# Meng-333/SRADSGAN

Measured on AMD Instinct MI355X. Metric: training images/sec (216x216, x4), higher is better.
Workload: dtype f32 (split-bf16 products: 3 bf16 MFMA terms per fp32 multiply, fp32 accumulate)

## Files before the change

### include/sradsgan_hip.h

```cpp
#ifndef SRADSGAN_HIP_H
#define SRADSGAN_HIP_H
#include <stddef.h>
#include <stdint.h>

#ifdef __cplusplus
extern "C" {
#endif

#define SRHIP_OK 0
#define SRHIP_ERR_ARG (-1)
#define SRHIP_ERR_LAUNCH (-2)
#define SRHIP_ERR_WORKSPACE (-3)

#define SRHIP_EPI_BIAS 1
#define SRHIP_EPI_LRELU 2
#define SRHIP_EPI_RESIDUAL 4
#define SRHIP_EPI_ROWSCALE 8
#define SRHIP_EPI_ACTMASK 32
#define SRHIP_EPI_CHANSCALE 16
#define SRHIP_EPI_GRADDATA 64

const char* srhip_last_error(void);
int srhip_abi_version(void);
int srhip_stream_fork(void* from_stream, void* to_stream);
// ... 178 lines not shown
size_t srhip_attn_tail_bwd_workspace(int n, int h, int w);
int srhip_attn_tail_bwd_spatial(const float* dz, const float* u, const float* s, const float* m, const float* pooled,
                                const int* argc, const float* w7, float* du, float* ds, float* dw7, int accumulate_dw7,
                                void* workspace, size_t workspace_bytes, int n, int h, int w, int c, void* stream);
size_t srhip_attn_tail_mlp_workspace(int n, int hidden);
int srhip_attn_tail_bwd_mlp(const float* ds, const float* avg, const float* mx, const float* s, const float* fc1,
                            const float* fc2, float* davg, float* dmax, float* dfc1, float* dfc2, int accumulate_dfc,
                            void* workspace, size_t workspace_bytes, int n, int c, int hidden, void* stream);
size_t srhip_attn_tail_bwd_fused_workspace(int n, int h, int w, int hidden);
int srhip_attn_tail_bwd(const float* dz, const float* u, const float* s, const float* m, const float* pooled, const int* argc,
                        const float* avg, const float* mx, const int* argmax_hw, const float* w7, const float* fc1,
                        const float* fc2, float* du, float* dw7, int accumulate_dw7, float* dfc1, float* dfc2,
                        int accumulate_dfc, void* workspace, size_t workspace_bytes, int n, int h, int w, int c, int hidden,
                        void* stream);
int srhip_attn_tail_bwd_pp(const float* dz, const float* u, const float* s, const float* m, const float* pooled, const int* argc,
                        const float* avg, const float* mx, const int* argmax_hw, const float* w7, const float* fc1,
                        const float* fc2, float* du, void* du_pp, float* dw7, int accumulate_dw7, float* dfc1, float* dfc2,
                        int accumulate_dfc, void* workspace, size_t workspace_bytes, int n, int h, int w, int c, int hidden,
                        void* stream);
int srhip_attn_tail_bwd_channel(float* du, const float* davg, const float* dmax, const int* argmax_hw, int n, int h,
                                int w, int c, void* stream);

size_t srhip_cgam_workspace(int n, int hw);
int srhip_cgam_fwd(const float* x, const float* gamma, float* y, float* att, void* workspace, size_t workspace_bytes,
                   int n, int hw, int c, void* stream);
int srhip_cgam_bwd(const float* dy, const float* x, const float* att, const float* gamma, float* dx, float* dgamma,
                   int accumulate_dgamma, void* workspace, size_t workspace_bytes, int n, int hw, int c, void* stream);
int srhip_sgam_flash_fwd(const float* q, const float* k, const float* v, const float* x, const float* gamma, float* y,
                         float* o, float* lse, int n, int hw, int dk, int c, void* stream);
size_t srhip_sgam_flash_bwd_workspace(int n, int hw);
int srhip_sgam_flash_bwd(const float* dy, const float* q, const float* k, const float* v, const float* o, const float* lse,
                         const float* gamma, float* dq, float* dk_out, float* dv, float* dgamma, int accumulate_dgamma,
                         void* workspace, size_t workspace_bytes, int n, int hw, int dk, int c, void* stream);

int srhip_cbam_pool_hw(const float* x, float* t, int* arg, int fixed_arg, int n, int hw, int c, void* stream);
int srhip_cbam_unpool_hw(const float* t, const int* arg, float* out, int n, int hw, int c, void* stream);
int srhip_cbam_pool_c(const float* x, float* t, int* argc, int fixed_arg, int n, int hw, int c, void* stream);
int srhip_cbam_unpool_c(const float* t, const int* argc, float* out, int n, int hw, int c, void* stream);
int srhip_cbam_scale(const float* x, const float* s, float* out, int n, int hw, int c, int mode, void* stream);
int srhip_cbam_dot(const float* a, const float* b, float* out, int n, int hw, int c, int mode, void* stream);
int srhip_sigmoid_fwd(const float* x, float* y, long count, int c, int pair, void* stream);
int srhip_sigmoid_bwd(const float* g, const float* y, float* dx, long count, int c, int pair, void* stream);
int srhip_sigmoid_bwd_bwd(const float* gg, const float* g, const float* y, float* dg, float* dy, long count, int c, int pair,
                          void* stream);

size_t srhip_reduce_workspace(void);
int srhip_l1_mean_fwd(const float* a, const float* b, float* out, void* workspace, size_t workspace_bytes, long count,
                      void* stream);
int srhip_l1_mean_bwd(const float* a, const float* b, const float* gout, float* da, float* db, long count, void* stream);
int srhip_mse_mean_fwd(const float* a, const float* b, float* out, void* workspace, size_t workspace_bytes, long count,
                       void* stream);
int srhip_mse_mean_bwd(const float* a, const float* b, const float* gout, float* da, float* db, long count, void* stream);
int srhip_smooth_l1_mean_fwd(const float* a, const float* b, float target, float* out, void* workspace, size_t workspace_bytes,
                             long count, void* stream);
int srhip_smooth_l1_mean_bwd(const float* a, const float* b, float target, const float* gout, float* da, float* db, long count,
                             void* stream);
int srhip_mean_fwd(const float* x, float* out, void* workspace, size_t workspace_bytes, long count, void* stream);
int srhip_mean_bwd(const float* gout, float* dx, long count, void* stream);
int srhip_gp_norm_penalty_fwd(const float* grads, float* out, void* workspace, size_t workspace_bytes, long npix, int c,
                              void* stream);
int srhip_gp_norm_penalty_bwd(const float* grads, const float* gout, float* dgrads, long npix, int c, void* stream);
#define SRHIP_GP_NORM_L2 0
#define SRHIP_GP_NORM_L1 1
#define SRHIP_GP_NORM_LINF 2
#define SRHIP_GP_PENALTY_LS 0
#define SRHIP_GP_PENALTY_HINGE 1
// ... 87 lines not shown
```

### sradsgan_amd/_hip.py

```python
import ctypes
import os

_HERE = os.path.dirname(os.path.abspath(__file__))
LIB_PATH = os.path.join(_HERE, 'lib', 'libsradsgan_hip.so')

_vp, _i, _f, _l, _sz = ctypes.c_void_p, ctypes.c_int, ctypes.c_float, ctypes.c_long, ctypes.c_size_t

SIGNATURES = {
    'srhip_last_error': (ctypes.c_char_p, []),
    'srhip_abi_version': (_i, []),
    'srhip_stream_fork': (_i, [_vp, _vp]),
    'srhip_debug_set': (_i, [_i, _i]),
    'srhip_probe_config': (_i, [_i] * 7),
    'srhip_probe_read': (_i, [_vp, _vp, _i]),
    'srhip_set_conv_math': (_i, [_i]),
    'srhip_get_conv_math': (_i, []),
    'srhip_resample_ksize': (_i, [_i, _i, _i]),
    'srhip_resample_coeffs': (_i, [_i, _i, _i, _vp, _vp]),
    'srhip_resample_pass_u8': (_i, [_vp, _vp, _vp, _vp, _i, _i, _i, _i, _i, _i, _i, _vp]),
    'srhip_u8_to_float': (_i, [_vp, _vp, _l, _vp]),
    'srhip_scene_tiles_u8': (_i, [_vp, _i, _i, _vp, _i, _i, _i, _vp, _vp]),
    'srhip_scene_blend_u8': (_i, [_vp, _i, _l, _l, _l] + [_vp] * 6 + [_i] * 8 + [_vp] * 3),
    'srhip_packed_elems': (_sz, [_i] * 5),
    'srhip_pack_entry_bytes': (_i, []),
# ... 23 lines not shown
    'srhip_conv2d_wgrad_pp_workspace': (_sz, [_i] * 8),
    'srhip_conv2d_wgrad_pp': (_i, [_i, _vp, _vp, _i, _i, _vp, _vp, _i, _vp, _sz] + [_i] * 6 + [_vp]),
    'srhip_conv2d_wgrad_act_ok': (_i, [_i] * 9),
    'srhip_conv2d_wgrad_act': (_i, [_vp] * 3 + [_f] + [_vp] * 3 + [_sz] + [_i] * 11 + [_vp]),
    'srhip_conv2d_wgrad': (_i, [_vp] * 6 + [_i, _vp, _sz] + [_i] * 11 + [_vp]),
    'srhip_colsum_workspace': (_sz, [_l, _i]),
    'srhip_colsum': (_i, [_vp, _vp, _vp, _sz, _l, _i, _i, _vp]),
    'srhip_lrelu_bwd': (_i, [_vp, _vp, _vp, _l, _f, _vp]),
    'srhip_lrelu_mask_bytes': (_sz, [_l]),
    'srhip_lrelu_bwd_bits': (_i, [_vp, _vp, _vp, _vp, _l, _f, _vp]),
    'srhip_maxpool2x2_fwd': (_i, [_vp, _vp, _i, _i, _i, _i, _vp]),
    'srhip_maxpool2x2_bwd': (_i, [_vp, _vp, _vp, _i, _i, _i, _i, _i, _vp]),
    'srhip_maxpool2x2_fwd_idx': (_i, [_vp, _vp, _vp, _i, _i, _i, _i, _vp]),
    'srhip_maxpool2x2_bwd_idx': (_i, [_vp, _vp, _vp, _i, _i, _i, _i, _i, _vp]),
    'srhip_pixel_shuffle_fwd': (_i, [_vp, _vp, _i, _i, _i, _i, _i, _f, _i, _vp]),
    'srhip_pixel_shuffle_bwd': (_i, [_vp, _vp, _vp, _i, _i, _i, _i, _i, _f, _i, _vp]),
    'srhip_attn_tail_workspace': (_sz, [_i]),
    'srhip_attn_tail_fwd': (_i, [_vp] * 12 + [_sz] + [_i] * 5 + [_vp]),
    'srhip_attn_tail_eval': (_i, [_vp] * 9 + [_sz] + [_i] * 5 + [_vp]),
    'srhip_attn_tail_bwd_workspace': (_sz, [_i] * 3),
    'srhip_attn_tail_bwd_spatial': (_i, [_vp] * 10 + [_i, _vp, _sz] + [_i] * 4 + [_vp]),
    'srhip_attn_tail_mlp_workspace': (_sz, [_i, _i]),
    'srhip_attn_tail_bwd_mlp': (_i, [_vp] * 10 + [_i, _vp, _sz] + [_i] * 3 + [_vp]),
    'srhip_attn_tail_bwd_fused_workspace': (_sz, [_i] * 4),
    'srhip_attn_tail_bwd': (_i, [_vp] * 14 + [_i] + [_vp] * 2 + [_i, _vp, _sz] + [_i] * 5 + [_vp]),
    'srhip_attn_tail_bwd_pp': (_i, [_vp] * 15 + [_i] + [_vp] * 2 + [_i, _vp, _sz] + [_i] * 5 + [_vp]),
    'srhip_attn_tail_bwd_channel': (_i, [_vp] * 4 + [_i] * 4 + [_vp]),
    'srhip_cgam_workspace': (_sz, [_i, _i]),
    'srhip_cgam_fwd': (_i, [_vp] * 5 + [_sz] + [_i] * 3 + [_vp]),
    'srhip_cgam_bwd': (_i, [_vp] * 6 + [_i, _vp, _sz] + [_i] * 3 + [_vp]),
    'srhip_sgam_flash_fwd': (_i, [_vp] * 8 + [_i] * 4 + [_vp]),
    'srhip_sgam_flash_bwd_workspace': (_sz, [_i, _i]),
    'srhip_sgam_flash_bwd': (_i, [_vp] * 11 + [_i, _vp, _sz] + [_i] * 4 + [_vp]),
    'srhip_cbam_pool_hw': (_i, [_vp, _vp, _vp, _i, _i, _i, _i, _vp]),
    'srhip_cbam_unpool_hw': (_i, [_vp, _vp, _vp, _i, _i, _i, _vp]),
    'srhip_cbam_pool_c': (_i, [_vp, _vp, _vp, _i, _i, _i, _i, _vp]),
    'srhip_cbam_unpool_c': (_i, [_vp, _vp, _vp, _i, _i, _i, _vp]),
    'srhip_cbam_scale': (_i, [_vp, _vp, _vp, _i, _i, _i, _i, _vp]),
    'srhip_cbam_dot': (_i, [_vp, _vp, _vp, _i, _i, _i, _i, _vp]),
    'srhip_sigmoid_fwd': (_i, [_vp, _vp, _l, _i, _i, _vp]),
    'srhip_sigmoid_bwd': (_i, [_vp, _vp, _vp, _l, _i, _i, _vp]),
    'srhip_sigmoid_bwd_bwd': (_i, [_vp] * 5 + [_l, _i, _i, _vp]),
    'srhip_reduce_workspace': (_sz, []),
    'srhip_l1_mean_fwd': (_i, [_vp] * 4 + [_sz, _l, _vp]),
    'srhip_l1_mean_bwd': (_i, [_vp] * 5 + [_l, _vp]),
    'srhip_mse_mean_fwd': (_i, [_vp] * 4 + [_sz, _l, _vp]),
    'srhip_mse_mean_bwd': (_i, [_vp] * 5 + [_l, _vp]),
    'srhip_smooth_l1_mean_fwd': (_i, [_vp, _vp, _f, _vp, _vp, _sz, _l, _vp]),
    'srhip_smooth_l1_mean_bwd': (_i, [_vp, _vp, _f] + [_vp] * 3 + [_l, _vp]),
    'srhip_mean_fwd': (_i, [_vp] * 3 + [_sz, _l, _vp]),
    'srhip_mean_bwd': (_i, [_vp] * 2 + [_l, _vp]),
    'srhip_gp_norm_penalty_fwd': (_i, [_vp] * 3 + [_sz, _l, _i, _vp]),
    'srhip_gp_norm_penalty_bwd': (_i, [_vp] * 3 + [_l, _i, _vp]),
    'srhip_gp_penalty_fwd': (_i, [_vp] * 3 + [_sz, _l, _i, _i, _i, _vp]),
    'srhip_gp_penalty_bwd': (_i, [_vp] * 3 + [_l, _i, _i, _i, _vp]),
    'srhip_bn_eval_fwd': (_i, [_vp] * 6 + [_l, _i, _f, _f, _i, _vp]),
    'srhip_dp_id_bytes': (_i, []),
    'srhip_dp_unique_id': (_i, [_vp]),
    'srhip_dp_init': (_i, [_vp, _i, _i]),
    'srhip_dp_world': (_i, []),
    'srhip_dp_rank': (_i, []),
    'srhip_dp_allreduce_bucket': (_i, [_vp, _sz, _vp]),
    'srhip_dp_broadcast': (_i, [_vp, _sz, _i, _vp]),
    'srhip_dp_finalize': (_i, []),
    'srhip_bn_workspace': (_sz, [_l, _i]),
    'srhip_bn_train_fwd': (_i, [_vp] * 9 + [_sz, _l, _i, _f, _f, _f, _i, _vp]),
# ... 109 lines not shown
```

### sradsgan_amd/csrc/global_attn.hip

```cpp
#include <math.h>

#include "common.h"

namespace srhip {

__device__ inline f32x16 ga_mfma(float a, float b, f32x16 c) { return __builtin_amdgcn_mfma_f32_32x32x2f32(a, b, c, 0, 0, 0); }
__device__ __forceinline__ int ga_row(int r, int h) { return (r & 3) + 8 * (r >> 2) + 4 * h; }

constexpr int GA_C = 64;
constexpr int GA_PIX = 128;
constexpr int GA_MS = 65;
constexpr int GA_VS = 68;
constexpr int GA_DK = 8;

__global__ __launch_bounds__(256) void ga_gram_partial_kernel(const float* __restrict__ a, const float* __restrict__ bm,
                                                              float* __restrict__ part, int hw, int nsplit) {
  const int split = blockIdx.x, img = blockIdx.y;
  const int lane = threadIdx.x & 63, wave = threadIdx.x >> 6;
  const int qi = wave >> 1, qj = wave & 1, h = lane >> 5, l31 = lane & 31;
  const int p0 = split * GA_PIX, p1 = min(p0 + GA_PIX, hw);
  const float* ab = a + (size_t)img * hw * GA_C + qi * 32 + l31;
  const float* bb = bm + (size_t)img * hw * GA_C + qj * 32 + l31;
  f32x16 acc;
#pragma unroll
  for (int r = 0; r < 16; ++r) acc[r] = 0.f;
  for (int p = p0; p < p1; p += 16) {
    float av[8], bv[8];
#pragma unroll
    for (int s = 0; s < 8; ++s) {
      const int pp = p + 2 * s + h;
      const bool ok = pp < p1;
      av[s] = ok ? ab[(size_t)pp * GA_C] : 0.f;
      bv[s] = ok ? bb[(size_t)pp * GA_C] : 0.f;
    }
#pragma unroll
// ... 793 lines not shown
    }
#pragma unroll
    for (int s = 0; s < 2; ++s) {
      ga_bf16x8 ph, pl;
      ga_split_regs(p, s, ph, pl);
#pragma unroll
      for (int u = 0; u < 2; ++u) {
        const int off = (32 * u + l31) * GA_TS + 16 * s + 8 * h;
        dvt[u] = ga_mma3(GA_FRAG(dth[b] + off), GA_FRAG(dtl[b] + off), ph, pl, dvt[u]);
      }
    }
#pragma unroll
    for (int r = 0; r < 16; ++r) p[r] = p[r] * (dp[r] - dd[r]);
#pragma unroll
    for (int s = 0; s < 2; ++s) {
      ga_bf16x8 sh, sl2;
      ga_split_regs(p, s, sh, sl2);
      const int off = (l31 & 7) * GA_TS + 16 * s + 8 * h;
      dkt = ga_mma3(GA_FRAG(qth[b] + off), GA_FRAG(qtl[b] + off), sh, sl2, dkt);
    }
    if (t + 1 < nt) store(b ^ 1);
    __syncthreads();
  }
  if (!kvalid) return;
  *reinterpret_cast<float4*>(dk + (base + kj) * GA_DK + 4 * h) = make_float4(dkt[0], dkt[1], dkt[2], dkt[3]);
#pragma unroll
  for (int u = 0; u < 2; ++u)
#pragma unroll
    for (int gq = 0; gq < 4; ++gq)
      *reinterpret_cast<float4*>(dv + (base + kj) * GA_C + 32 * u + 8 * gq + 4 * h) =
          make_float4(dvt[u][4 * gq], dvt[u][4 * gq + 1], dvt[u][4 * gq + 2], dvt[u][4 * gq + 3]);
}

int g_sgam_cfg = 0;
static inline bool ga_split_math() { return g_conv_math >= 1 && g_sgam_cfg != 1; }

static inline int ga_nsplit(int hw) { return cdiv(hw, GA_PIX); }
static inline int ga_prep_blocks(long npix) {
  long b = (npix + 15) / 16;
  return (int)(b < 1 ? 1 : (b > 1024 ? 1024 : b));
}

}

using namespace srhip;

extern "C" {

size_t srhip_cgam_workspace(int n, int hw) {
  if (n <= 0 || hw <= 0) return 0;
  return ((size_t)n * ga_nsplit(hw) * GA_C * GA_C + (size_t)n * GA_C * GA_C + (size_t)n + 64) * sizeof(float);
}

int srhip_cgam_fwd(const float* x, const float* gamma, float* y, float* att, void* workspace, size_t workspace_bytes,
                   int n, int hw, int c, void* stream) {
  SRHIP_REQUIRE(c == GA_C, "cgam_fwd: C must be 64 (sradsgan.py:194), got %d", c);
  SRHIP_REQUIRE(n > 0 && hw > 0, "cgam_fwd: empty input");
  SRHIP_REQUIRE((((uintptr_t)x | (uintptr_t)y | (uintptr_t)att) & 15) == 0, "cgam_fwd: pointers must be 16-byte aligned");
  if (!workspace || workspace_bytes < srhip_cgam_workspace(n, hw)) {
    set_error("cgam_fwd: workspace %zu bytes < required %zu", workspace_bytes, srhip_cgam_workspace(n, hw));
    return SRHIP_ERR_WORKSPACE;
  }
  hipStream_t st = as_stream(stream);
  const int ns = ga_nsplit(hw);
  float* part = static_cast<float*>(workspace);
  hipLaunchKernelGGL(ga_gram_partial_kernel, dim3(ns, n), dim3(256), 0, st, x, x, part, hw, ns);
// ... 41 lines not shown
  const long npix = (long)n * hw;
  return ((size_t)npix + (size_t)ga_prep_blocks(npix) + 64) * sizeof(float);
}

int srhip_sgam_flash_bwd(const float* dy, const float* q, const float* k, const float* v, const float* o, const float* lse,
                         const float* gamma, float* dq, float* dk_, float* dv, float* dgamma, int accumulate_dgamma,
                         void* workspace, size_t workspace_bytes, int n, int hw, int dk, int c, void* stream) {
  SRHIP_REQUIRE(c == GA_C && dk == GA_DK, "sgam_flash_bwd: C must be 64 and q/k channels 8, got %d / %d", c, dk);
  SRHIP_REQUIRE(n > 0 && hw > 0, "sgam_flash_bwd: empty input");
  SRHIP_REQUIRE((((uintptr_t)q | (uintptr_t)k | (uintptr_t)v | (uintptr_t)dy | (uintptr_t)o | (uintptr_t)dq | (uintptr_t)dk_ | (uintptr_t)dv) & 15) == 0,
                "sgam_flash_bwd: pointers must be 16-byte aligned");
  if (!workspace || workspace_bytes < srhip_sgam_flash_bwd_workspace(n, hw)) {
    set_error("sgam_flash_bwd: workspace %zu bytes < required %zu", workspace_bytes, srhip_sgam_flash_bwd_workspace(n, hw));
    return SRHIP_ERR_WORKSPACE;
  }
  hipStream_t st = as_stream(stream);
  const long npix = (long)n * hw;
  const int pb = ga_prep_blocks(npix);
  float* rowdot = static_cast<float*>(workspace);
  float* dgpart = rowdot + npix;
  hipLaunchKernelGGL(ga_sgam_bwd_prep_kernel, dim3(pb), dim3(256), 0, st, dy, o, rowdot, dgpart, npix);
  if (dgamma) hipLaunchKernelGGL(ga_sum_small_kernel, dim3(1), dim3(64), 0, st, dgpart, pb, dgamma, accumulate_dgamma);
  const dim3 grid(cdiv(hw, GA_PIX), n);
  if (ga_split_math()) {
    hipLaunchKernelGGL(ga_sgam_bwd_dq_x3_kernel, grid, dim3(256), 0, st, q, k, v, dy, lse, rowdot, gamma, dq, hw);
    hipLaunchKernelGGL(ga_sgam_bwd_dkv_x3_kernel, grid, dim3(256), 0, st, q, k, v, dy, lse, rowdot, gamma, dk_, dv, hw);
  } else {
    hipLaunchKernelGGL(ga_sgam_bwd_dq_kernel, grid, dim3(256), 0, st, q, k, v, dy, lse, rowdot, gamma, dq, hw);
    hipLaunchKernelGGL(ga_sgam_bwd_dkv_kernel, grid, dim3(256), 0, st, q, k, v, dy, lse, rowdot, gamma, dk_, dv, hw);
  }
  return check_launch("sgam_flash_bwd");
}

}
```

### sradsgan_amd/ops.py

```python
import contextlib
import ctypes
import os
import threading
import weakref
from typing import NamedTuple

import torch
from torch.autograd import Function

from . import _hip

EPI_BIAS, EPI_LRELU, EPI_RESIDUAL, EPI_ROWSCALE, EPI_CHANSCALE, EPI_GRADDATA = 1, 2, 4, 8, 16, 64
CL = torch.channels_last

class _State:
    skip_param_grads = False
    wgrads = None
    skip_ids = frozenset()
    stop_ids = frozenset()
    capturing = False
    last_out_pp = None
    carry = None
    carry_expect = None
    carry_token = 0
# ... 1577 lines not shown

    @staticmethod
    def backward(ctx, dy):
        x, att, gamma = ctx.saved_tensors
        dy = nhwc(dy)
        n, c, h, w = x.shape
        lib = _hip.lib()
        dx = torch.empty_like(x, memory_format=CL)
        skip = _skip_param_grads(gamma) or not ctx.needs_input_grad[1]
        dgam, acc = (None, 0) if skip else _gamma_slot(gamma)
        ws = _ws(lib.srhip_cgam_workspace(n, h * w), x)
        gam = gamma.detach().reshape(1).contiguous()
        _hip.check(lib.srhip_cgam_bwd(_p(dy), _p(x), _p(att), _p(gam), _p(dx), _p(dgam), acc, _p(ws), ws.numel() * 4,
                                      n, h * w, c, _stream()), 'cgam_bwd')
        return dx, (None if (skip or acc) else dgam.view(gamma.shape))


def cgam(x, gamma):
    return _Cgam.apply(x, gamma)


class _SgamCore(Function):

    @staticmethod
    def forward(ctx, x, q, k, v, gamma):
        _require_gpu(x, 'sgam')
        x, q, k, v = nhwc(x), nhwc(q), nhwc(k), nhwc(v)
        n, c, h, w = x.shape
        lib = _hip.lib()
        y = torch.empty_like(x, memory_format=CL)
        o = torch.empty_like(x, memory_format=CL)
        lse = torch.empty(n, h * w, device=x.device, dtype=torch.float32)
        gam = gamma.detach().reshape(1).contiguous()
        _hip.check(lib.srhip_sgam_flash_fwd(_p(q), _p(k), _p(v), _p(x), _p(gam), _p(y), _p(o), _p(lse), n, h * w,
                                            q.shape[1], c, _stream()), 'sgam_flash_fwd')
        ctx.save_for_backward(q, k, v, o, lse, gamma)
        return y

    @staticmethod
    def backward(ctx, dy):
        q, k, v, o, lse, gamma = ctx.saved_tensors
        dy = nhwc(dy)
        n, c, h, w = v.shape
        lib = _hip.lib()
        dq, dk = torch.empty_like(q, memory_format=CL), torch.empty_like(k, memory_format=CL)
        dv = torch.empty_like(v, memory_format=CL)
        skip = _skip_param_grads(gamma) or not ctx.needs_input_grad[4]
        dgam, acc = (None, 0) if skip else _gamma_slot(gamma)
        ws = _ws(lib.srhip_sgam_flash_bwd_workspace(n, h * w), v)
        gam = gamma.detach().reshape(1).contiguous()
        _hip.check(lib.srhip_sgam_flash_bwd(_p(dy), _p(q), _p(k), _p(v), _p(o), _p(lse), _p(gam), _p(dq), _p(dk), _p(dv),
                                            _p(dgam), acc, _p(ws), ws.numel() * 4, n, h * w, q.shape[1], c, _stream()),
                   'sgam_flash_bwd')
        return _passed_through(dy), dq, dk, dv, (None if (skip or acc) else dgam.view(gamma.shape))


def sgam(x, q, k, v, gamma):
    return _SgamCore.apply(x, q, k, v, gamma)


def _bn_reference_bwd(dy, x, y, gamma, eps, slope):
    n = x.numel() // x.shape[1]
    dz = dy if slope is None else dy * torch.where(y > 0, 1.0, float(slope))
    mean = x.mean((0, 2, 3), keepdim=True)
    var = x.var((0, 2, 3), unbiased=False, keepdim=True)
    invstd = torch.rsqrt(var + eps)
    xhat = (x - mean) * invstd
    dbeta = dz.sum((0, 2, 3))
    dgamma = (dz * xhat).sum((0, 2, 3))
    dx = (gamma.view(1, -1, 1, 1) * invstd) * (dz - dbeta.view(1, -1, 1, 1) / n - xhat * dgamma.view(1, -1, 1, 1) / n)
    return dx, dgamma, dbeta


_BN_BWD_X = os.environ.get('SRHIP_BN_BWD_X', '1') == '1'
_BN_FOLD = os.environ.get('SRHIP_BN_FOLD', '1') == '1'


@contextlib.contextmanager
def bn_fold_second_order():
    if not _BN_FOLD:
        yield
        return
    prev, _state.bn_fold = getattr(_state, 'bn_fold', None), {}
    ok = False
    try:
        yield
# ... 1322 lines not shown
```

Before: 673.6.

## Stage pre-split K/V tile images via LDS DMA in spatial attention kernels

Adds a pre-pass that packs each 32-pixel key/value tile into a contiguous global "image" holding both the fp32 data and the bf16 hi/lo split operands. The spatial-attention forward and backward kernels then stream these images into LDS with double-buffered buffer-load DMA, instead of each block re-splitting and transposing K/V itself. The intent is to drop the redundant per-block split/transpose work and to overlap global loads with MFMA compute. The cost is extra workspace, extra image-build launches and more global traffic for the packed tiles.

```diff
diff --git a/include/sradsgan_hip.h b/include/sradsgan_hip.h
--- a/include/sradsgan_hip.h
+++ b/include/sradsgan_hip.h
@@ -234,6 +234,14 @@
 int srhip_sgam_flash_bwd(const float* dy, const float* q, const float* k, const float* v, const float* o, const float* lse,
                          const float* gamma, float* dq, float* dk_out, float* dv, float* dgamma, int accumulate_dgamma,
                          void* workspace, size_t workspace_bytes, int n, int hw, int dk, int c, void* stream);
+size_t srhip_sgam_staged_fwd_workspace(int n, int hw);
+int srhip_sgam_staged_fwd(const float* q, const float* k, const float* v, const float* x, const float* gamma, float* y,
+                          float* o, float* lse, void* workspace, size_t workspace_bytes, int n, int hw, int dk, int c,
+                          void* stream);
+size_t srhip_sgam_staged_bwd_workspace(int n, int hw);
+int srhip_sgam_staged_bwd(const float* dy, const float* q, const float* k, const float* v, const float* o, const float* lse,
+                          const float* gamma, float* dq, float* dk_out, float* dv, float* dgamma, int accumulate_dgamma,
+                          void* workspace, size_t workspace_bytes, int n, int hw, int dk, int c, void* stream);
 
 int srhip_cbam_pool_hw(const float* x, float* t, int* arg, int fixed_arg, int n, int hw, int c, void* stream);
 int srhip_cbam_unpool_hw(const float* t, const int* arg, float* out, int n, int hw, int c, void* stream);
diff --git a/sradsgan_amd/_hip.py b/sradsgan_amd/_hip.py
--- a/sradsgan_amd/_hip.py
+++ b/sradsgan_amd/_hip.py
@@ -79,6 +79,10 @@
     'srhip_sgam_flash_fwd': (_i, [_vp] * 8 + [_i] * 4 + [_vp]),
     'srhip_sgam_flash_bwd_workspace': (_sz, [_i, _i]),
     'srhip_sgam_flash_bwd': (_i, [_vp] * 11 + [_i, _vp, _sz] + [_i] * 4 + [_vp]),
+    'srhip_sgam_staged_fwd_workspace': (_sz, [_i, _i]),
+    'srhip_sgam_staged_fwd': (_i, [_vp] * 9 + [_sz] + [_i] * 4 + [_vp]),
+    'srhip_sgam_staged_bwd_workspace': (_sz, [_i, _i]),
+    'srhip_sgam_staged_bwd': (_i, [_vp] * 11 + [_i, _vp, _sz] + [_i] * 4 + [_vp]),
     'srhip_cbam_pool_hw': (_i, [_vp, _vp, _vp, _i, _i, _i, _i, _vp]),
     'srhip_cbam_unpool_hw': (_i, [_vp, _vp, _vp, _i, _i, _i, _vp]),
     'srhip_cbam_pool_c': (_i, [_vp, _vp, _vp, _i, _i, _i, _i, _vp]),
diff --git a/sradsgan_amd/csrc/global_attn.hip b/sradsgan_amd/csrc/global_attn.hip
--- a/sradsgan_amd/csrc/global_attn.hip
+++ b/sradsgan_amd/csrc/global_attn.hip
@@ -1,6 +1,7 @@
 #include <math.h>
 
 #include "common.h"
+#include "conv_dev.h"
 
 namespace srhip {
 
@@ -860,6 +861,338 @@
           make_float4(dvt[u][4 * gq], dvt[u][4 * gq + 1], dvt[u][4 * gq + 2], dvt[u][4 * gq + 3]);
 }
 
+constexpr int GI_KT = 0;
+constexpr int GF_VTH = 1024, GF_VTL = GF_VTH + GA_C * GA_TS * 2, GF_TILE = GF_VTL + GA_C * GA_TS * 2;
+constexpr int GQ_KTH = 1024, GQ_KTL = GQ_KTH + GA_DK * GA_TS * 2, GQ_VRH = GQ_KTL + GA_DK * GA_TS * 2,
+              GQ_VRL = GQ_VRH + 32 * GA_RS * 2, GQ_END = GQ_VRL + 32 * GA_RS * 2, GQ_TILE = 12288;
+constexpr int GK_QTH = 1024, GK_QTL = GK_QTH + GA_DK * GA_TS * 2, GK_LT = GK_QTL + GA_DK * GA_TS * 2, GK_DT = GK_LT + 128,
+              GK_DRH = GK_DT + 128, GK_DRL = GK_DRH + 32 * GA_RS * 2, GK_DTH = GK_DRL + 32 * GA_RS * 2,
+              GK_DTL = GK_DTH + GA_C * GA_TS * 2, GK_END = GK_DTL + GA_C * GA_TS * 2, GK_TILE = 22528;
+static_assert(GF_TILE % 1024 == 0 && GQ_TILE % 1024 == 0 && GK_TILE % 1024 == 0, "a wave's DMA moves 1 KB");
+static_assert(GQ_END <= GQ_TILE && GK_END <= GK_TILE, "image layout");
+
+template <int KIND>
+__global__ __launch_bounds__(256) void ga_sgam_image_kernel(const float* __restrict__ wide, const float* __restrict__ narrow,
+                                                            const float* __restrict__ lse, const float* __restrict__ rowdot,
+                                                            const float* __restrict__ gamma, char* __restrict__ out, int hw) {
+  constexpr int TILE = KIND == 0 ? GF_TILE : (KIND == 1 ? GQ_TILE : GK_TILE);
+  __shared__ __attribute__((aligned(16))) char im[TILE];
+  const int t = blockIdx.x, img = blockIdx.y, tid = threadIdx.x, nt = gridDim.x;
+  const size_t base = (size_t)img * hw;
+  for (int i = tid * 16; i < TILE; i += 256 * 16) *reinterpret_cast<uint4*>(im + i) = make_uint4(0u, 0u, 0u, 0u);
+  __syncthreads();
+  const float g = KIND == 2 ? gamma[0] : 1.f;
+  GaStage st_;
+  ga_stage_load(st_, wide, narrow, base, t * 32, hw, tid, g);
+  float* nt_ = reinterpret_cast<float*>(im + GI_KT);
+  if constexpr (KIND == 0) {
+    ga_store_wide_T(st_, reinterpret_cast<__bf16*>(im + GF_VTH), reinterpret_cast<__bf16*>(im + GF_VTL), tid);
+    ga_store_narrow(st_, nt_, nullptr, nullptr, tid);
+  } else if constexpr (KIND == 1) {
+    ga_store_wide_R(st_, reinterpret_cast<__bf16*>(im + GQ_VRH), reinterpret_cast<__bf16*>(im + GQ_VRL), tid);
+    ga_store_narrow(st_, nt_, reinterpret_cast<__bf16*>(im + GQ_KTH), reinterpret_cast<__bf16*>(im + GQ_KTL), tid);
+  } else {
+    ga_store_wide_R(st_, reinterpret_cast<__bf16*>(im + GK_DRH), reinterpret_cast<__bf16*>(im + GK_DRL), tid);
+    ga_store_wide_T(st_, reinterpret_cast<__bf16*>(im + GK_DTH), reinterpret_cast<__bf16*>(im + GK_DTL), tid);
+    ga_store_narrow(st_, nt_, reinterpret_cast<__bf16*>(im + GK_QTH), reinterpret_cast<__bf16*>(im + GK_QTL), tid);
+    if (tid >= 64 && tid < 96) {
+      const int row = t * 32 + tid - 64;
+      reinterpret_cast<float*>(im + GK_LT)[tid - 64] = row < hw ? lse[base + row] : INFINITY;
+    } else if (tid >= 96 && tid < 128) {
+      const int row = t * 32 + tid - 96;
+      reinterpret_cast<float*>(im + GK_DT)[tid - 96] = row < hw ? g * rowdot[base + row] : 0.f;
+    }
+  }
+  __syncthreads();
+  char* o = out + ((size_t)img * nt + t) * TILE;
+  for (int i = tid * 16; i < TILE; i += 256 * 16) *reinterpret_cast<uint4*>(o + i) = *reinterpret_cast<const uint4*>(im + i);
+}
+
+template <int NCH>
+__device__ __forceinline__ void ga_issue_stage(__amdgpu_buffer_rsrc_t rs, unsigned goff, unsigned ldst, int wave) {
+#pragma unroll
+  for (int j = 0; j < (NCH + 3) / 4; ++j) {
+    const int c = wave + 4 * j;
+    if (4 * j + 3 < NCH || c < NCH) lds_dma16_buf(goff + (unsigned)c * 1024u, rs, ldst + (unsigned)c * 1024u);
+  }
+}
+__device__ __forceinline__ void ga_stage_sync() {
+  wait_vmcnt<0>();
+  __builtin_amdgcn_s_barrier();
+  asm volatile("" ::: "memory");
+}
+
+__global__ __launch_bounds__(256) void ga_sgam_fwd_st_kernel(const float* __restrict__ q, const char* __restrict__ image,
+                                                             const float* __restrict__ x, const float* __restrict__ gamma,
+                                                             float* __restrict__ y, float* __restrict__ osave,
+                                                             float* __restrict__ lse, int hw) {
+  constexpr int STAGE = 2 * GF_TILE;
+  __shared__ __attribute__((aligned(1024))) char lds[2 * STAGE];
+  const unsigned lds_base = (unsigned)(size_t)(__attribute__((address_space(3))) char*)lds;
+  const int img = blockIdx.y, tid = threadIdx.x, lane = tid & 63, h = lane >> 5, l31 = lane & 31;
+  const int wave = __builtin_amdgcn_readfirstlane(tid >> 6);
+  const size_t base = (size_t)img * hw;
+  const int qi = blockIdx.x * GA_PIX + wave * 32 + l31;
+  const bool qvalid = qi < hw;
+  const float4 qf = qvalid ? *reinterpret_cast<const float4*>(q + (base + qi) * GA_DK + 4 * h) : make_float4(0.f, 0.f, 0.f, 0.f);
+  const int nt = (hw + 31) >> 5, ns = (nt + 1) >> 1;
+  __amdgpu_buffer_rsrc_t rs = __builtin_amdgcn_make_buffer_rsrc(const_cast<char*>(image) + (size_t)img * nt * GF_TILE, 0,
+                                                                (unsigned)nt * GF_TILE, 0x00020000);
+  ga_issue_stage<STAGE / 1024>(rs, lane * 16u, lds_base, wave);
+  f32x16 ot[2];
+#pragma unroll
+  for (int u = 0; u < 2; ++u)
+#pragma unroll
+    for (int r = 0; r < 16; ++r) ot[u][r] = 0.f;
+  float m = -INFINITY, l = 0.f;
+  asm volatile("" ::"v"(qf.x), "v"(qf.y), "v"(qf.z), "v"(qf.w));
+  for (int s = 0; s < ns; ++s) {
+    ga_stage_sync();
+    if (s + 1 < ns) ga_issue_stage<STAGE / 1024>(rs, (unsigned)(s + 1) * STAGE + lane * 16u, lds_base + ((s + 1) & 1) * STAGE, wave);
+#pragma unroll
+    for (int sub = 0; sub < 2; ++sub) {
+      const int t = 2 * s + sub, k0 = t * 32;
+      if (t < nt) {
+        const char* tb = lds + (s & 1) * STAGE + sub * GF_TILE;
+        const __bf16* vth = reinterpret_cast<const __bf16*>(tb + GF_VTH);
+        const __bf16* vtl = reinterpret_cast<const __bf16*>(tb + GF_VTL);
+        f32x16 p = ga_scores_t(reinterpret_cast<const float*>(tb + GI_KT), qf, h, l31);
+        if (k0 + 32 > hw) {
+#pragma unroll
+          for (int r = 0; r < 16; ++r)
+            if (k0 + ga_row(r, h) >= hw) p[r] = -INFINITY;
+        }
+        float tmax = -INFINITY;
+#pragma unroll
+        for (int r = 0; r < 16; ++r) tmax = fmaxf(tmax, p[r]);
+        tmax = fmaxf(tmax, __shfl_xor(tmax, 32, 64));
+        const float mnew = fmaxf(m, tmax);
+        const float alpha = ga_exp(m - mnew);
+        m = mnew;
+        float psum = 0.f;
+#pragma unroll
+        for (int r = 0; r < 16; ++r) {
+          p[r] = ga_exp(p[r] - mnew);
+          psum += p[r];
+        }
+        if (__builtin_amdgcn_ballot_w64(alpha != 1.0f) != 0) {
+          l = l * alpha + psum;
+#pragma unroll
+          for (int u = 0; u < 2; ++u)
+#pragma unroll
+            for (int r = 0; r < 16; ++r) ot[u][r] *= alpha;
+        } else {
+          l = l + psum;
+        }
+#pragma unroll
+        for (int s2 = 0; s2 < 2; ++s2) {
+          ga_bf16x8 ph, pl;
+          ga_split_regs(p, s2, ph, pl);
+#pragma unroll
+          for (int u = 0; u < 2; ++u) {
+            const int off = (32 * u + l31) * GA_TS + 16 * s2 + 8 * h;
+            ot[u] = ga_mma3(GA_FRAG(vth + off), GA_FRAG(vtl + off), ph, pl, ot[u]);
+          }
+        }
+      }
+    }
+  }
+  l += __shfl_xor(l, 32, 64);
+  if (!qvalid) return;
+  const float inv = 1.f / l, g = gamma[0];
+  if (h == 0) lse[base + qi] = m + logf(l);
+#pragma unroll
+  for (int u = 0; u < 2; ++u)
+#pragma unroll
+    for (int gq = 0; gq < 4; ++gq) {
+      const size_t idx = (base + qi) * GA_C + 32 * u + 8 * gq + 4 * h;
+      const float4 o4 = make_float4(ot[u][4 * gq] * inv, ot[u][4 * gq + 1] * inv, ot[u][4 * gq + 2] * inv, ot[u][4 * gq + 3] * inv);
+      const float4 x4 = *reinterpret_cast<const float4*>(x + idx);
+      *reinterpret_cast<float4*>(osave + idx) = o4;
+      *reinterpret_cast<float4*>(y + idx) = make_float4(g * o4.x + x4.x, g * o4.y + x4.y, g * o4.z + x4.z, g * o4.w + x4.w);
+    }
+}
+
+__global__ __launch_bounds__(256) void ga_sgam_bwd_dq_st_kernel(const float* __restrict__ q, const char* __restrict__ image,
+                                                                const float* __restrict__ dy, const float* __restrict__ lse,
+                                                                const float* __restrict__ rowdot, const float* __restrict__ gamma,
+                                                                float* __restrict__ dq, int hw) {
+  constexpr int STAGE = 2 * GQ_TILE;
+  __shared__ __attribute__((aligned(1024))) char lds[2 * STAGE];
+  const unsigned lds_base = (unsigned)(size_t)(__attribute__((address_space(3))) char*)lds;
+  const int img = blockIdx.y, tid = threadIdx.x, lane = tid & 63, h = lane >> 5, l31 = lane & 31;
+  const int wave = __builtin_amdgcn_readfirstlane(tid >> 6);
+  const size_t base = (size_t)img * hw;
+  const int qi = blockIdx.x * GA_PIX + wave * 32 + l31;
+  const bool qvalid = qi < hw;
+  const float g = gamma[0];
+  const float4 z4 = make_float4(0.f, 0.f, 0.f, 0.f);
+  const float4 qf = qvalid ? *reinterpret_cast<const float4*>(q + (base + qi) * GA_DK + 4 * h) : z4;
+  const float lq = qvalid ? lse[base + qi] : 0.f;
+  const float dq_ = qvalid ? g * rowdot[base + qi] : 0.f;
+  ga_bf16x8 doh[4], dol[4];
+#pragma unroll
+  for (int c = 0; c < 4; ++c) {
+    const float* dr = dy + (base + (qvalid ? qi : 0)) * GA_C + 16 * c + 8 * h;
+    float4 a = *reinterpret_cast<const float4*>(dr), b = *reinterpret_cast<const float4*>(dr + 4);
+    if (!qvalid) a = b = z4;
+    a.x *= g; a.y *= g; a.z *= g; a.w *= g;
+    b.x *= g; b.y *= g; b.z *= g; b.w *= g;
+    ga_split_f4x2(a, b, doh[c], dol[c]);
+  }
+  const int nt = (hw + 31) >> 5, ns = (nt + 1) >> 1;
+  __amdgpu_buffer_rsrc_t rs = __builtin_amdgcn_make_buffer_rsrc(const_cast<char*>(image) + (size_t)img * nt * GQ_TILE, 0,
+                                                                (unsigned)nt * GQ_TILE, 0x00020000);
+  ga_issue_stage<STAGE / 1024>(rs, lane * 16u, lds_base, wave);
+  f32x16 dqt;
+#pragma unroll
+  for (int r = 0; r < 16; ++r) dqt[r] = 0.f;
+  for (int s = 0; s < ns; ++s) {
+    ga_stage_sync();
+    if (s + 1 < ns) ga_issue_stage<STAGE / 1024>(rs, (unsigned)(s + 1) * STAGE + lane * 16u, lds_base + ((s + 1) & 1) * STAGE, wave);
+#pragma unroll
+    for (int sub = 0; sub < 2; ++sub) {
+      const int t = 2 * s + sub, k0 = t * 32;
+      if (t < nt) {
+        const char* tb = lds + (s & 1) * STAGE + sub * GQ_TILE;
+        const float* kt = reinterpret_cast<const float*>(tb + GI_KT);
+        const __bf16* kth = reinterpret_cast<const __bf16*>(tb + GQ_KTH);
+        const __bf16* ktl = reinterpret_cast<const __bf16*>(tb + GQ_KTL);
+        const __bf16* vrh = reinterpret_cast<const __bf16*>(tb + GQ_VRH);
+        const __bf16* vrl = reinterpret_cast<const __bf16*>(tb + GQ_VRL);
+        f32x16 p = ga_scores_t(kt, qf, h, l31);
+        if (k0 + 32 > hw) {
+#pragma unroll
+          for (int r = 0; r < 16; ++r) p[r] = (k0 + ga_row(r, h) < hw) ? ga_exp(p[r] - lq) : 0.f;
+        } else {
+#pragma unroll
+          for (int r = 0; r < 16; ++r) p[r] = ga_exp(p[r] - lq);
+        }
+        f32x16 dpt;
+#pragma unroll
+        for (int r = 0; r < 16; ++r) dpt[r] = 0.f;
+#pragma unroll
+        for (int c = 0; c < 4; ++c) {
+          const int off = l31 * GA_RS + 16 * c + 8 * h;
+          dpt = ga_mma3(GA_FRAG(vrh + off), GA_FRAG(vrl + off), doh[c], dol[c], dpt);
+        }
+#pragma unroll
+        for (int r = 0; r < 16; ++r) p[r] = p[r] * (dpt[r] - dq_);
+#pragma unroll
+        for (int s2 = 0; s2 < 2; ++s2) {
+          ga_bf16x8 sh, sl;
+          ga_split_regs(p, s2, sh, sl);
+          const int off = (l31 & 7) * GA_TS + 16 * s2 + 8 * h;
+          dqt = ga_mma3(GA_FRAG(kth + off), GA_FRAG(ktl + off), sh, sl, dqt);
+        }
+      }
+    }
+  }
+  if (qvalid) *reinterpret_cast<float4*>(dq + (base + qi) * GA_DK + 4 * h) = make_float4(dqt[0], dqt[1], dqt[2], dqt[3]);
+}
+
+__global__ __launch_bounds__(256) __attribute__((amdgpu_waves_per_eu(3, 3))) void ga_sgam_bwd_dkv_st_kernel(const float* __restrict__ k, const float* __restrict__ v,
+                                                                 const char* __restrict__ image, float* __restrict__ dk,
+                                                                 float* __restrict__ dv, int hw) {
+  constexpr int STAGE = GK_TILE;
+  __shared__ __attribute__((aligned(1024))) char lds[2 * STAGE];
+  const unsigned lds_base = (unsigned)(size_t)(__attribute__((address_space(3))) char*)lds;
+  const int img = blockIdx.y, tid = threadIdx.x, lane = tid & 63, h = lane >> 5, l31 = lane & 31;
+  const int wave = __builtin_amdgcn_readfirstlane(tid >> 6);
+  const size_t base = (size_t)img * hw;
+  const int kj = blockIdx.x * GA_PIX + wave * 32 + l31;
+  const bool kvalid = kj < hw;
+  const float4 z4 = make_float4(0.f, 0.f, 0.f, 0.f);
+  const float4 kf = kvalid ? *reinterpret_cast<const float4*>(k + (base + kj) * GA_DK + 4 * h) : z4;
+  ga_bf16x8 vfh[4], vfl[4];
+#pragma unroll
+  for (int c = 0; c < 4; ++c) {
+    const float* vr = v + (base + (kvalid ? kj : 0)) * GA_C + 16 * c + 8 * h;
+    float4 a = *reinterpret_cast<const float4*>(vr), b = *reinterpret_cast<const float4*>(vr + 4);
+    if (!kvalid) a = b = z4;
+    ga_split_f4x2(a, b, vfh[c], vfl[c]);
+  }
+  const int nt = (hw + 31) >> 5;
+  __amdgpu_buffer_rsrc_t rs = __builtin_amdgcn_make_buffer_rsrc(const_cast<char*>(image) + (size_t)img * nt * GK_TILE, 0,
+                                                                (unsigned)nt * GK_TILE, 0x00020000);
+  ga_issue_stage<STAGE / 1024>(rs, lane * 16u, lds_base, wave);
+  f32x16 dvt[2], dkt;
+#pragma unroll
+  for (int r = 0; r < 16; ++r) {
+    dvt[0][r] = 0.f;
+    dvt[1][r] = 0.f;
+    dkt[r] = 0.f;
+  }
+  for (int t = 0; t < nt; ++t) {
+    ga_stage_sync();
+    if (t + 1 < nt) ga_issue_stage<STAGE / 1024>(rs, (unsigned)(t + 1) * STAGE + lane * 16u, lds_base + ((t + 1) & 1) * STAGE, wave);
+    const char* tb = lds + (t & 1) * STAGE;
+    const float* qt = reinterpret_cast<const float*>(tb + GI_KT);
+    const __bf16* qth = reinterpret_cast<const __bf16*>(tb + GK_QTH);
+    const __bf16* qtl = reinterpret_cast<const __bf16*>(tb + GK_QTL);
+    const float* lt = reinterpret_cast<const float*>(tb + GK_LT);
+    const float* dt = reinterpret_cast<const float*>(tb + GK_DT);
+    const __bf16* drh = reinterpret_cast<const __bf16*>(tb + GK_DRH);
+    const __bf16* drl = reinterpret_cast<const __bf16*>(tb + GK_DRL);
+    const __bf16* dth = reinterpret_cast<const __bf16*>(tb + GK_DTH);
+    const __bf16* dtl = reinterpret_cast<const __bf16*>(tb + GK_DTL);
+    const float4 q4 = *reinterpret_cast<const float4*>(qt + l31 * GA_DK + 4 * h);
+    f32x16 p;
+#pragma unroll
+    for (int r = 0; r < 16; ++r) p[r] = 0.f;
+    p = ga_mfma(q4.x, kf.x, p);
+    p = ga_mfma(q4.y, kf.y, p);
+    p = ga_mfma(q4.z, kf.z, p);
+    p = ga_mfma(q4.w, kf.w, p);
+    float dd[16];
+#pragma unroll
+    for (int gq = 0; gq < 4; ++gq) {
+      const float4 l4 = *reinterpret_cast<const float4*>(lt + 8 * gq + 4 * h);
+      const float4 d4 = *reinterpret_cast<const float4*>(dt + 8 * gq + 4 * h);
+      p[4 * gq] = ga_exp(p[4 * gq] - l4.x);
+      p[4 * gq + 1] = ga_exp(p[4 * gq + 1] - l4.y);
+      p[4 * gq + 2] = ga_exp(p[4 * gq + 2] - l4.z);
+      p[4 * gq + 3] = ga_exp(p[4 * gq + 3] - l4.w);
+      dd[4 * gq] = d4.x; dd[4 * gq + 1] = d4.y; dd[4 * gq + 2] = d4.z; dd[4 * gq + 3] = d4.w;
+    }
+    f32x16 dp;
+#pragma unroll
+    for (int r = 0; r < 16; ++r) dp[r] = 0.f;
+#pragma unroll
+    for (int c = 0; c < 4; ++c) {
+      const int off = l31 * GA_RS + 16 * c + 8 * h;
+      dp = ga_mma3(GA_FRAG(drh + off), GA_FRAG(drl + off), vfh[c], vfl[c], dp);
+    }
+#pragma unroll
+    for (int s = 0; s < 2; ++s) {
+      ga_bf16x8 ph, pl;
+      ga_split_regs(p, s, ph, pl);
+#pragma unroll
+      for (int u = 0; u < 2; ++u) {
+        const int off = (32 * u + l31) * GA_TS + 16 * s + 8 * h;
+        dvt[u] = ga_mma3(GA_FRAG(dth + off), GA_FRAG(dtl + off), ph, pl, dvt[u]);
+      }
+    }
+#pragma unroll
+    for (int r = 0; r < 16; ++r) p[r] = p[r] * (dp[r] - dd[r]);
+#pragma unroll
+    for (int s = 0; s < 2; ++s) {
+      ga_bf16x8 sh, sl2;
+      ga_split_regs(p, s, sh, sl2);
+      const int off = (l31 & 7) * GA_TS + 16 * s + 8 * h;
+      dkt = ga_mma3(GA_FRAG(qth + off), GA_FRAG(qtl + off), sh, sl2, dkt);
+    }
+  }
+  if (!kvalid) return;
+  *reinterpret_cast<float4*>(dk + (base + kj) * GA_DK + 4 * h) = make_float4(dkt[0], dkt[1], dkt[2], dkt[3]);
+#pragma unroll
+  for (int u = 0; u < 2; ++u)
+#pragma unroll
+    for (int gq = 0; gq < 4; ++gq)
+      *reinterpret_cast<float4*>(dv + (base + kj) * GA_C + 32 * u + 8 * gq + 4 * h) =
+          make_float4(dvt[u][4 * gq], dvt[u][4 * gq + 1], dvt[u][4 * gq + 2], dvt[u][4 * gq + 3]);
+}
+
 int g_sgam_cfg = 0;
 static inline bool ga_split_math() { return g_conv_math >= 1 && g_sgam_cfg != 1; }
 
@@ -967,4 +1300,73 @@
   return check_launch("sgam_flash_bwd");
 }
 
-}
+static inline size_t ga_image_bytes(int n, int hw, int tile) { return (size_t)n * cdiv(hw, 32) * tile; }
+static inline size_t ga_round256(size_t b) { return (b + 255) & ~(size_t)255; }
+static inline bool ga_staged() { return ga_split_math() && g_sgam_cfg != 2; }
+
+size_t srhip_sgam_staged_fwd_workspace(int n, int hw) {
+  if (n <= 0 || hw <= 0) return 0;
+  return ga_image_bytes(n, hw, GF_TILE) + 256;
+}
+
+int srhip_sgam_staged_fwd(const float* q, const float* k, const float* v, const float* x, const float* gamma, float* y,
+                          float* o, float* lse, void* workspace, size_t workspace_bytes, int n, int hw, int dk, int c,
+                          void* stream) {
+  if (!ga_staged()) return srhip_sgam_flash_fwd(q, k, v, x, gamma, y, o, lse, n, hw, dk, c, stream);
+  SRHIP_REQUIRE(c == GA_C && dk == GA_DK, "sgam_staged_fwd: C must be 64 and q/k channels 8 (sradsgan.py:157-159), got %d / %d", c, dk);
+  SRHIP_REQUIRE(n > 0 && hw > 0, "sgam_staged_fwd: empty input");
+  SRHIP_REQUIRE((((uintptr_t)q | (uintptr_t)k | (uintptr_t)v | (uintptr_t)x | (uintptr_t)y | (uintptr_t)o | (uintptr_t)workspace) & 15) == 0,
+                "sgam_staged_fwd: pointers must be 16-byte aligned");
+  SRHIP_REQUIRE((size_t)cdiv(hw, 32) * GK_TILE < ((size_t)1 << 31), "sgam_staged_fwd: image of %d pixels exceeds 32-bit tile offsets", hw);
+  if (!workspace || workspace_bytes < srhip_sgam_staged_fwd_workspace(n, hw)) {
+    set_error("sgam_staged_fwd: workspace %zu bytes < required %zu", workspace_bytes, srhip_sgam_staged_fwd_workspace(n, hw));
+    return SRHIP_ERR_WORKSPACE;
+  }
+  hipStream_t st = as_stream(stream);
+  char* image = static_cast<char*>(workspace);
+  hipLaunchKernelGGL(ga_sgam_image_kernel<0>, dim3(cdiv(hw, 32), n), dim3(256), 0, st, v, k, (const float*)nullptr,
+                     (const float*)nullptr, gamma, image, hw);
+  hipLaunchKernelGGL(ga_sgam_fwd_st_kernel, dim3(cdiv(hw, GA_PIX), n), dim3(256), 0, st, q, (const char*)image, x, gamma, y, o, lse, hw);
+  return check_launch("sgam_staged_fwd");
+}
+
+size_t srhip_sgam_staged_bwd_workspace(int n, int hw) {
+  if (n <= 0 || hw <= 0) return 0;
+  return ga_round256(srhip_sgam_flash_bwd_workspace(n, hw)) + ga_round256(ga_image_bytes(n, hw, GQ_TILE)) +
+         ga_image_bytes(n, hw, GK_TILE) + 256;
+}
+
+int srhip_sgam_staged_bwd(const float* dy, const float* q, const float* k, const float* v, const float* o, const float* lse,
+                          const float* gamma, float* dq, float* dk_, float* dv, float* dgamma, int accumulate_dgamma,
+                          void* workspace, size_t workspace_bytes, int n, int hw, int dk, int c, void* stream) {
+  if (!workspace || workspace_bytes < srhip_sgam_staged_bwd_workspace(n, hw)) {
+    set_error("sgam_staged_bwd: workspace %zu bytes < required %zu", workspace_bytes, srhip_sgam_staged_bwd_workspace(n, hw));
+    return SRHIP_ERR_WORKSPACE;
+  }
+  if (!ga_staged())
+    return srhip_sgam_flash_bwd(dy, q, k, v, o, lse, gamma, dq, dk_, dv, dgamma, accumulate_dgamma, workspace, workspace_bytes,
+                                n, hw, dk, c, stream);
+  SRHIP_REQUIRE(c == GA_C && dk == GA_DK, "sgam_staged_bwd: C must be 64 and q/k channels 8, got %d / %d", c, dk);
+  SRHIP_REQUIRE(n > 0 && hw > 0, "sgam_staged_bwd: empty input");
+  SRHIP_REQUIRE((((uintptr_t)q | (uintptr_t)k | (uintptr_t)v | (uintptr_t)dy | (uintptr_t)o | (uintptr_t)dq | (uintptr_t)dk_ | (uintptr_t)dv |
+                  (uintptr_t)workspace) & 15) == 0,
+                "sgam_staged_bwd: pointers must be 16-byte aligned");
+  SRHIP_REQUIRE((size_t)cdiv(hw, 32) * GK_TILE < ((size_t)1 << 31), "sgam_staged_bwd: image of %d pixels exceeds 32-bit tile offsets", hw);
+  hipStream_t st = as_stream(stream);
+  const long npix = (long)n * hw;
+  const int pb = ga_prep_blocks(npix);
+  float* rowdot = static_cast<float*>(workspace);
+  float* dgpart = rowdot + npix;
+  char* qimage = static_cast<char*>(workspace) + ga_round256(srhip_sgam_flash_bwd_workspace(n, hw));
+  char* kimage = qimage + ga_round256(ga_image_bytes(n, hw, GQ_TILE));
+  hipLaunchKernelGGL(ga_sgam_bwd_prep_kernel, dim3(pb), dim3(256), 0, st, dy, o, rowdot, dgpart, npix);
+  if (dgamma) hipLaunchKernelGGL(ga_sum_small_kernel, dim3(1), dim3(64), 0, st, dgpart, pb, dgamma, accumulate_dgamma);
+  const dim3 tiles(cdiv(hw, 32), n), grid(cdiv(hw, GA_PIX), n);
+  hipLaunchKernelGGL(ga_sgam_image_kernel<1>, tiles, dim3(256), 0, st, v, k, (const float*)nullptr, (const float*)nullptr, gamma, qimage, hw);
+  hipLaunchKernelGGL(ga_sgam_image_kernel<2>, tiles, dim3(256), 0, st, dy, q, lse, (const float*)rowdot, gamma, kimage, hw);
+  hipLaunchKernelGGL(ga_sgam_bwd_dq_st_kernel, grid, dim3(256), 0, st, q, (const char*)qimage, dy, lse, (const float*)rowdot, gamma, dq, hw);
+  hipLaunchKernelGGL(ga_sgam_bwd_dkv_st_kernel, grid, dim3(256), 0, st, k, v, (const char*)kimage, dk_, dv, hw);
+  return check_launch("sgam_staged_bwd");
+}
+
+}
diff --git a/sradsgan_amd/ops.py b/sradsgan_amd/ops.py
--- a/sradsgan_amd/ops.py
+++ b/sradsgan_amd/ops.py
@@ -1633,8 +1633,9 @@
         o = torch.empty_like(x, memory_format=CL)
         lse = torch.empty(n, h * w, device=x.device, dtype=torch.float32)
         gam = gamma.detach().reshape(1).contiguous()
-        _hip.check(lib.srhip_sgam_flash_fwd(_p(q), _p(k), _p(v), _p(x), _p(gam), _p(y), _p(o), _p(lse), n, h * w,
-                                            q.shape[1], c, _stream()), 'sgam_flash_fwd')
+        ws = _ws(lib.srhip_sgam_staged_fwd_workspace(n, h * w), v)
+        _hip.check(lib.srhip_sgam_staged_fwd(_p(q), _p(k), _p(v), _p(x), _p(gam), _p(y), _p(o), _p(lse), _p(ws), ws.numel() * 4,
+                                             n, h * w, q.shape[1], c, _stream()), 'sgam_staged_fwd')
         ctx.save_for_backward(q, k, v, o, lse, gamma)
         return y
 
@@ -1648,11 +1649,11 @@
         dv = torch.empty_like(v, memory_format=CL)
         skip = _skip_param_grads(gamma) or not ctx.needs_input_grad[4]
         dgam, acc = (None, 0) if skip else _gamma_slot(gamma)
-        ws = _ws(lib.srhip_sgam_flash_bwd_workspace(n, h * w), v)
+        ws = _ws(lib.srhip_sgam_staged_bwd_workspace(n, h * w), v)
         gam = gamma.detach().reshape(1).contiguous()
-        _hip.check(lib.srhip_sgam_flash_bwd(_p(dy), _p(q), _p(k), _p(v), _p(o), _p(lse), _p(gam), _p(dq), _p(dk), _p(dv),
-                                            _p(dgam), acc, _p(ws), ws.numel() * 4, n, h * w, q.shape[1], c, _stream()),
-                   'sgam_flash_bwd')
+        _hip.check(lib.srhip_sgam_staged_bwd(_p(dy), _p(q), _p(k), _p(v), _p(o), _p(lse), _p(gam), _p(dq), _p(dk), _p(dv),
+                                             _p(dgam), acc, _p(ws), ws.numel() * 4, n, h * w, q.shape[1], c, _stream()),
+                   'sgam_staged_bwd')
         return _passed_through(dy), dq, dk, dv, (None if (skip or acc) else dgam.view(gamma.shape))
 
 
```

Result: no change. 679.9 (median of 6 runs) (+0.9%).
